# thomasantony/splat

Hardware: AMD Instinct MI355X
Metric: frames_per_sec (higher is better)
Workload: dtype f32

## Files before the change

### splat_amd/csrc/splat_api.hip

```cpp
#include <algorithm>
#include <cmath>
#include <cstdio>
#include <cstdlib>
#include <cstring>
#include <mutex>
#include <new>
#include <string>
#include <unordered_map>
#include <vector>

#include "splat_context.h"

using namespace splat;

static thread_local std::string g_create_error;
static std::mutex g_ledger_mu;
static std::unordered_map<void*, std::pair<splat_ctx*, size_t>> g_ledger;

namespace splat {
CommState** ctx_comm_slot(splat_ctx* c) { return &c->comm; }
hipStream_t ctx_stream(splat_ctx* c) { return c->stream; }
hipStream_t frame_stream(splat_ctx* c) { return (c->last_lane && c->comp2) ? c->comp2 : c->stream; }
int frame_tail(splat_ctx* c) {
    if (c->last_ring < 0 || !c->ring[c->last_ring].used) return SPLAT_OK;
// ... 502 lines not shown
            c->iters_alloc = m * 4u;
        }
        HIP_TRY(c, hipMemsetAsync(c->d_iters, 0, sizeof(uint2) * (size_t)m * 4u, cs));
        iters = c->d_iters;
        c->iters_valid = true;
    }
    CompositeArgs comp{};
    comp.s = cs; comp.knobs = &c->knobs; comp.n_tiles = m; comp.fc = c->fc; comp.recs = s.recs; comp.argb = d_argb; comp.status = f.d_st; comp.orig = c->orig;
    comp.fused_sort_max = retained ? 0u : c->fused_sort_max; comp.iters = iters; comp.keep_keys = want_iters || f.retain == SPLAT_RETAIN_WRITER;
    comp.pair_walk = pd.pair_walk != 0;
    comp.libm_exp = (c->cfg.mode & SPLAT_MODE_LIBM_EXP) != 0; comp.clear_first = c->clear_first;
    comp.lists = f.lists; comp.lists.near_m = pd.near_cap ? s.near_m : nullptr;
    comp.keys = f.keys; comp.keys.keys2 = pd.comp_sorts != 0 ? s.keys2 : nullptr;
    if (retained) {
        const bool near = c->ret_set.near_cap != 0u;
        comp.lists.near_m = near ? s.near_m : nullptr; comp.keys.keys2 = near ? s.keys2 : nullptr;
    }
    comp.hints = hint_table(c);
    if (c->knobs.dbg_stage_cache != 0u && f.retain == SPLAT_RETAIN_WRITER) {
        const size_t waves = (size_t)c->m_alloc * 4u;
        if (!c->stage_nv || !c->stage_mask) {
            dfree(c->stage_nv); dfree(c->stage_mask);
            HIP_TRY(c, dmalloc(c, &c->stage_nv, sizeof(unsigned int) * 2u * waves));
            HIP_TRY(c, dmalloc(c, &c->stage_mask, sizeof(unsigned long long) * 32u * waves));
        }
        HIP_TRY(c, hipMemsetAsync(c->stage_nv, 0, sizeof(unsigned int) * 2u * waves, cs));
        c->ret_set.frames = 0;
    }
    if (retained && c->knobs.dbg_stage_cache != 0u && c->stage_nv && c->stage_mask) {
        comp.stage_nv = c->stage_nv; comp.stage_mask = c->stage_mask;
        if (c->knobs.dbg_proven_starts != 0u && c->fc.close_width == 0.0f) comp.proven_start = c->proven_start();
        if (c->knobs.dbg_stage_cache == 2u && c->ret_set.frames >= 2u)
            HIP_TRY(c, hipMemsetAsync(c->stage_mask, 0, sizeof(unsigned long long) * 32u * (size_t)c->m_alloc * 4u, cs));
        c->ret_set.frames++;
    }
    comp.refine = c->fc.close_width == 0.0f ? pd.refine : 0u;
    launch_composite(comp);
    c->last_near = retained ? c->ret_set.near_cap != 0u : pd.near_cap != 0u;
    HIP_TRY(c, f.mark(6, cs));
    if (want_iters) HIP_TRY(c, hipMemcpyAsync(&c->h_status[f.r], f.d_st, sizeof(FrameStatus), hipMemcpyDeviceToHost, cs));
    HIP_TRY(c, hipEventRecord(f.ev->e[7], cs));
    return SPLAT_OK;
}

int decide_retention(splat_ctx* c, const splat_camera* cam, int* action) {
    splat_retain_input in;
    std::memset(&in, 0, sizeof in);
    static_assert(sizeof(splat_camera) + 2 * sizeof(int32_t) <= sizeof in.cam, "the camera and the slab fit the decision's words");
    std::memcpy(in.cam, cam, sizeof(splat_camera));
    const int32_t slab[2] = {c->slab0, c->slab1};
    std::memcpy(reinterpret_cast<unsigned char*>(in.cam) + sizeof(splat_camera), slab, sizeof slab);
    in.epoch = c->bin_epoch; in.still_frames = c->pol.still_frames;
    in.enabled = (c->retain_lists != 0 && c->knobs.dbg_ntiles == 0u) ? 1 : 0;
    in.overlap = c->overlap; in.one_pass = c->fc.bucket_cap ? 1 : 0;
    splat_retain_decision d;
    const int wr = c->ret_set.ring;
// ... 431 lines not shown
    option_from_env(c, SPLAT_OPT_HOST_ZERO_COPY, "SPLAT_HOST_ZERO_COPY", 0, 1);
    option_from_env(c, SPLAT_OPT_COUNT_FIRST, "SPLAT_COUNT_FIRST", 0, 2);
    if (const char* kg = std::getenv("SPLAT_KEYS_PER_GAUSSIAN")) {
        const int v = std::atoi(kg);
        c->keys_per_gaussian = v <= 0 ? 0u : (unsigned int)std::min(256, std::max(4, v));
        c->env_pinned |= 1u << SPLAT_OPT_KEYS_PER_GAUSSIAN;
    }
    option_from_env(c, SPLAT_OPT_LARGE_SPLAT_TILES, "SPLAT_LARGE_TILES", -1, 1048576);
    option_from_env(c, SPLAT_OPT_LARGE_LIST_MIN, "SPLAT_LARGE_LIST_MIN", -1, 1e9);
    option_from_env(c, SPLAT_OPT_START_REFINE, "SPLAT_START_REFINE", 0, 1);
    option_from_env(c, SPLAT_OPT_RETAIN_LISTS, "SPLAT_RETAIN", 0, 1);
    if (const char* lm = std::getenv("SPLAT_LAYOUT_MOTION")) c->layout_motion = std::atoi(lm) != 0 ? 1 : 0;
    if (const char* k1 = std::getenv("SPLAT_SORT_RADIX_MIN")) c->knobs.sort_radix_min = (unsigned int)std::max(0, std::atoi(k1));
    if (const char* k2 = std::getenv("SPLAT_SCAN_THREADS")) c->knobs.scan_threads = std::atoi(k2);
    if (const char* k3 = std::getenv("SPLAT_DBG_NTILES")) c->knobs.dbg_ntiles = (unsigned int)std::max(0, std::atoi(k3));
    if (const char* k8 = std::getenv("SPLAT_DBG_SELECT_STRIDE")) c->knobs.dbg_select_stride = (unsigned int)std::max(0, std::atoi(k8));
    if (const char* k10 = std::getenv("SPLAT_START_HINTS")) { c->start_hints = std::min(2, std::max(0, std::atoi(k10))); c->env_pinned |= 1u << SPLAT_OPT_START_HINTS; }
    if (const char* k7 = std::getenv("SPLAT_DBG_ONE_PASS_SELECT")) c->one_pass_select = std::atoi(k7) != 0;
    if (const char* k11 = std::getenv("SPLAT_DBG_KEYS2_ENTRIES")) c->knobs.dbg_keys2_entries = std::strtoull(k11, nullptr, 10);
    if (const char* k9 = std::getenv("SPLAT_DBG_HINT_RADIUS")) c->knobs.dbg_hint_radius = std::atoi(k9);
    if (const char* k12 = std::getenv("SPLAT_DBG_SELECT_BLIND")) c->knobs.dbg_select_blind = std::atoi(k12) != 0 ? 1u : 0u;
    if (const char* k15 = std::getenv("SPLAT_DBG_PROVEN_STARTS")) c->knobs.dbg_proven_starts = (unsigned int)std::min(2, std::max(0, std::atoi(k15)));
    if (const char* k14 = std::getenv("SPLAT_DBG_BRACKET_COUNT")) c->knobs.dbg_bracket_count = std::atoi(k14) != 0 ? 1u : 0u;
    if (const char* k13 = std::getenv("SPLAT_DBG_STAGE_CACHE")) c->knobs.dbg_stage_cache = (unsigned int)std::min(2, std::max(0, std::atoi(k13)));
    if (const char* k5 = std::getenv("SPLAT_DBG_STARTS")) c->knobs.dbg_starts = std::atoi(k5) != 0 ? 1u : 0u;
    if (const char* k4 = std::getenv("SPLAT_COMP_LDS_PAD")) c->knobs.comp_lds_pad = (unsigned int)std::max(0, std::atoi(k4));
    if (const char* k1p = std::getenv("SPLAT_K1_LDS_PAD")) c->knobs.k1_lds_pad = (unsigned int)std::min(48 * 1024, std::max(0, std::atoi(k1p)));
    auto bail = [&](const char* what, hipError_t err) {
        g_create_error = std::string(what) + ": " + hipGetErrorString(err);
        splat_destroy(c);
        return SPLAT_ERR_HIP;
    };
    if ((e = hipSetDevice(cfg->device)) != hipSuccess) return bail("hipSetDevice", e);
    if ((e = init_device_kernels()) != hipSuccess) return bail("hipFuncSetAttribute", e);
    if ((e = hipStreamCreateWithFlags(&c->stream, hipStreamNonBlocking)) != hipSuccess) return bail("hipStreamCreate", e);
    c->own_stream = true;
    {
        int lo = 0, hi = 0;
        (void)hipDeviceGetStreamPriorityRange(&lo, &hi);
        int prio = c->pipeline >= 6 ? (lo + hi) / 2 : hi;
        if (const char* ep = std::getenv("SPLAT_BIN_PRIO")) prio = std::atoi(ep) > 0 ? hi : (std::atoi(ep) < 0 ? lo : (lo + hi) / 2);
        if ((e = hipStreamCreateWithPriority(&c->bin_stream, hipStreamNonBlocking, prio)) != hipSuccess) return bail("hipStreamCreate", e);
        if ((e = hipStreamCreateWithPriority(&c->sort_stream, hipStreamNonBlocking, prio)) != hipSuccess) return bail("hipStreamCreate", e);
    }
    if (c->overlap >= 2 && c->pipeline) { if ((e = ensure_copy_stream(c)) != hipSuccess) return bail("hipStreamCreate", e); c->comp2 = c->copy_stream; }
    for (Slot& s : c->slots) {
// ... 624 lines not shown
```

### splat_amd/csrc/splat_context.h

```cpp
#ifndef SPLAT_CONTEXT_H
#define SPLAT_CONTEXT_H
#include <string>
#include <vector>

#include "splat_internal.h"
#include "../../include/splat_policy.h"
#include "../../include/splat_retain.h"

#define HIP_TRY(ctx, expr)                                                                             \
    do {                                                                                               \
        hipError_t _e = (expr);                                                                        \
        if (_e != hipSuccess) {                                                                        \
            (ctx)->err = std::string(#expr) + ": " + hipGetErrorString(_e);                            \
            return SPLAT_ERR_HIP;                                                                      \
        }                                                                                              \
    } while (0)

namespace splat {
constexpr int N_EV = 9;
constexpr int N_TIMES = 6;
constexpr int EV_RING = 32;
static_assert(EV_RING == SPLAT_POLICY_RING, "the frame policy sees the whole status ring");
constexpr int N_SLOTS = 4;

// ... 93 lines not shown
    uint64_t bucket_bytes = 128ull << 30;
    uint64_t layout_want = 0;
    unsigned int layout_m = 0;
    bool last_one_pass = false;
    unsigned int* zero_layout = nullptr;
    uint64_t dev_bytes = 0, dev_bytes_peak = 0;
    splat::LaunchKnobs knobs;
    float region_spare = 4.0f;
    uint64_t frame_idx = 0;
    uint64_t bin_idx = 0;
    int retain_lists = 1;
    uint64_t bin_epoch = 0;
    splat_retain_state ret{};
    uint64_t frames_retained = 0;
    struct RetainSet {
        int slot = -1, ring = -1;
        unsigned int near_cap = 0;
        splat::FrameStatus status{};
        unsigned int frames = 0;
    } ret_set;
    unsigned int* stage_nv = nullptr;
    unsigned long long* stage_mask = nullptr;
    unsigned int* proven_start() const { return stage_nv ? stage_nv + (size_t)m_alloc * 4u : nullptr; }
    int last_slot = -1;
    bool last_lists_in_memory = false;
    splat::FrameStatus* h_status = nullptr;
    splat::FrameStatus* d_status_ring = nullptr;
    bool clear_first = false;
    uint32_t* d_img = nullptr;
    size_t img_cap = 0;
    static constexpr int S_IMGS = 4;
    uint32_t* s_img[S_IMGS] = {};
    size_t s_cap = 0;
    hipStream_t copy_stream = nullptr;
    hipEvent_t s_rendered[S_IMGS] = {}, s_copied[S_IMGS] = {};
    const uint32_t* s_dst[S_IMGS] = {};
    bool s_used[S_IMGS] = {};
    uint64_t s_idx = 0;
    int s_ring[S_IMGS] = {-1, -1, -1, -1};
    splat_camera s_cam[S_IMGS] = {};
    int slab0 = 0, slab1 = -1;
    splat::EvSet ring[splat::EV_RING];
    int ring_next = 0;
    int last_ring = -1;
    double acc_ms[splat::N_TIMES] = {0, 0, 0, 0, 0, 0};
    uint64_t acc_frames = 0;
// ... 58 lines not shown
```

### splat_amd/csrc/splat_device_math.h

```cpp
#pragma once
#include <hip/hip_runtime.h>
#include <math.h>

__host__ __device__ __forceinline__ float reject_threshold(float opacity) {
    return (opacity > 0.0f) ? (logf(1.0f / (255.0f * opacity)) - 1e-3f)
                            : ((opacity <= 0.0f) ? 3.0e38f : -3.0e38f);
}

__host__ __device__ __forceinline__ bool any_sample_covered(float c, float h, float lo, float hi, float off) {
    float s1 = fminf(fmaxf(floorf(c - off) + off, lo), hi);
    float s2 = fminf(s1 + 1.0f, hi);
    return (int)(fabsf(s1 - c) <= h) | (int)(fabsf(s2 - c) <= h);
}

__device__ __forceinline__ float exp_neg(float x) {
    const float L2E_HI = __uint_as_float(0x3fb8aa3bu), L2E_LO = __uint_as_float(0x32a5705fu);
    const float LN2 = 0.6931471805599453f;
    float ph = x * L2E_HI;
    float pl = fmaf(x, L2E_HI, -ph);
    pl = fmaf(x, L2E_LO, pl);
    const float e = __builtin_amdgcn_exp2f(ph);
    return fmaf(e * pl, LN2, e);
}

// ... 44 lines not shown
    const unsigned long long ki = __builtin_bit_cast(unsigned long long, kd);
    kd -= SHIFT;
    const double r = fma(InvLn2N, xd, -kd);
    const double sc = __builtin_bit_cast(double, tab[ki & 31ull] + (ki << 47));
    const double zz = C0 * r + C1;
    const double r2 = r * r;
    double y = C2 * r + 1.0;
    y = zz * r2 + y;
    y = y * sc;
    return (float)y;
}
__host__ __device__ __forceinline__ float sigmoid_libm(float v) { return 1.0f / (1.0f + expf_libm_full(-v)); }

__host__ __device__ __forceinline__ float div255(float k) {
    const float RH = 0x1.010102p-8f, RL = -0x1.fdfdfep-33f;
    return fmaf(k, RH, k * RL);
}
__device__ __forceinline__ float blend_channel(float k, float ia, float ac) {
    const float x = __builtin_amdgcn_fmed3f(ia * div255(k) + ac, 0.0f, 1.0f);
    return truncf(x * 255.0f);
}

template <class E>
__device__ __forceinline__ float fragment_alpha(float sx, float sy, const float4& a, const float4& b, E e_of_power, bool& cov) {
    float dx = sx - a.x, dy = a.y - sy;
    cov = (fabsf(dx) <= a.z) & (fabsf(dy) <= a.w);
    float power = -0.5f * (b.x * dx * dx + b.z * dy * dy) - b.y * dx * dy;
    float alpha = fminf(0.99f, b.w * e_of_power(power));
    bool accept = cov & !(power > 0.0f) & !(alpha < 1.0f / 255.0f);
    return accept ? alpha : 0.0f;
}

typedef float f2 __attribute__((ext_vector_type(2)));
__device__ __forceinline__ f2 pk_add_clamp(f2 a, f2 b) {
    f2 r;
    asm("v_pk_add_f32 %0, %1, %2 clamp" : "=v"(r) : "v"(a), "v"(b));
    return r;
}
__device__ __forceinline__ f2 blend_channel2(f2 k, float ia, f2 ac) {
    const float RH = 0x1.010102p-8f, RL = -0x1.fdfdfep-33f;
    const f2 f = __builtin_elementwise_fma(k, (f2)(RH), k * RL);
    const f2 y = pk_add_clamp(ia * f, ac) * 255.0f;
    return (f2){truncf(y.x), truncf(y.y)};
}
__device__ __forceinline__ f2 exp_neg2(f2 power) {
    const float L2E_HI = __uint_as_float(0x3fb8aa3bu), L2E_LO = __uint_as_float(0x32a5705fu), LN2 = 0.6931471805599453f;
    const f2 ph = power * L2E_HI;
    f2 pl = __builtin_elementwise_fma(power, (f2)(L2E_HI), -ph);
    pl = __builtin_elementwise_fma(power, (f2)(L2E_LO), pl);
    const f2 e = {__builtin_amdgcn_exp2f(ph.x), __builtin_amdgcn_exp2f(ph.y)};
    return __builtin_elementwise_fma(e * pl, (f2)(LN2), e);
}
__device__ __forceinline__ f2 fragment_alpha2(f2 sx2, f2 sy2, f2 cx, f2 cy, const float4& h, f2 A, f2 C, f2 Bc, f2 op) {
// ... 11 lines not shown
```

### splat_amd/csrc/splat_internal.h

```cpp
#ifndef SPLAT_INTERNAL_H
#define SPLAT_INTERNAL_H
#include <hip/hip_runtime.h>
#include <stdint.h>

#include "../../include/splat_hip.h"

#ifndef SPLAT_K1X
#define SPLAT_K1X 0
#endif
#ifndef SPLAT_EXP_STAGE2
#define SPLAT_EXP_STAGE2 0
#endif
#ifndef SPLAT_EXP_NO_BRACKET
#define SPLAT_EXP_NO_BRACKET 0
#endif
#ifndef SPLAT_EXP_K1DUMMY
#define SPLAT_EXP_K1DUMMY 0
#endif
#ifndef SPLAT_EXP_SKIPFULL
#define SPLAT_EXP_SKIPFULL 0
#endif
#ifndef SPLAT_EXP_SORT2
#define SPLAT_EXP_SORT2 0
#endif
// ... 64 lines not shown
    unsigned long long layout_total;
};

struct Rec {
    float4 a;
    float4 b;
    float4 c;
};

struct LaunchKnobs {
    unsigned int sort_radix_min = 128;
    int scan_threads = 0;
    unsigned int dbg_ntiles = 0;
    unsigned int comp_lds_pad = 0;
    unsigned int k1_lds_pad = 0;
    unsigned int dbg_select_stride = 0;
    unsigned long long dbg_keys2_entries = 0;
    int dbg_hint_radius = -1;
    unsigned int dbg_select_blind = 0;
    unsigned int dbg_starts = 0;
    unsigned int dbg_bracket_count = 0;
    unsigned int dbg_proven_starts = 1;
    unsigned int dbg_stage_cache = 1;
};

struct HintTable {
    unsigned int* base;
    size_t stride;

    static constexpr unsigned int NEED_PLANE = 0u, NEED_PLANES = 4u;
    static constexpr unsigned int DEPTH_PLANE = NEED_PLANE + NEED_PLANES, DEPTH_PLANES = 1u;
    static constexpr unsigned int START_PLANE = DEPTH_PLANE + DEPTH_PLANES, START_PLANES = 4u;
    static constexpr unsigned int REFINE_PLANE = START_PLANE + START_PLANES, REFINE_PLANES = 4u;
    static constexpr unsigned int HINT_WORDS = 13u;
    static_assert(DEPTH_PLANE == 4u && START_PLANE == 5u && REFINE_PLANE == 9u && REFINE_PLANE + REFINE_PLANES == HINT_WORDS,
                  "the four parts tile the table exactly");

    unsigned int* plane(unsigned int k) const { return base ? base + k * stride : nullptr; }
    unsigned int* needs() const { return plane(NEED_PLANE); }
    unsigned int* select_depth() const { return plane(DEPTH_PLANE); }
    unsigned int* starts() const { return plane(START_PLANE); }
    unsigned int* refinement() const { return plane(REFINE_PLANE); }
    size_t words() const { return HINT_WORDS * stride; }
    size_t bytes() const { return sizeof(unsigned int) * words(); }
};

// ... 158 lines not shown
    unsigned int tiles_x, tile_rows;
    unsigned int grid;
    bool at_rest;
    int hint_radius;
};
void launch_select(const SelectArgs& a);

struct CompositeArgs {
    hipStream_t s; const LaunchKnobs* knobs; unsigned int n_tiles; FrameConst fc;
    TileLists lists;
    KeyBuffers keys;
    const Rec* recs; uint32_t* argb; FrameStatus* status; const unsigned int* orig;
    unsigned int fused_sort_max;
    uint2* iters;
    bool keep_keys;
    bool pair_walk;
    bool libm_exp;
    bool clear_first;
    HintTable hints;
    unsigned int refine;
    unsigned int* proven_start;
    unsigned int* stage_nv;
    unsigned long long* stage_mask;
};
void launch_composite(const CompositeArgs& a);
void launch_status_set(hipStream_t s, FrameStatus* status, const FrameStatus& v);
hipError_t init_device_kernels();

struct CommState;
CommState** ctx_comm_slot(splat_ctx* c);
hipStream_t ctx_stream(splat_ctx* c);
hipStream_t frame_stream(splat_ctx* c);
int ctx_device(const splat_ctx* c);
int frame_tail(splat_ctx* c);
int ctx_quiesce(splat_ctx* c);
int ctx_fail(splat_ctx* c, int code, const char* msg);
void comm_release(CommState* s);

}
#endif
```

### splat_amd/csrc/splat_kernels.hip

```cpp
#include <algorithm>
#include <cstddef>
#include <cstdlib>
#include <type_traits>

#include "splat_internal.h"
#include "splat_device_math.h"

namespace splat {
static constexpr unsigned long long KERNELS_EXP2F_TAB[32] = {
    0x3ff0000000000000ull, 0x3fefd9b0d3158574ull, 0x3fefb5586cf9890full, 0x3fef9301d0125b51ull, 0x3fef72b83c7d517bull,
    0x3fef54873168b9aaull, 0x3fef387a6e756238ull, 0x3fef1e9df51fdee1ull, 0x3fef06fe0a31b715ull, 0x3feef1a7373aa9cbull,
    0x3feedea64c123422ull, 0x3feece086061892dull, 0x3feebfdad5362a27ull, 0x3feeb42b569d4f82ull, 0x3feeab07dd485429ull,
    0x3feea47eb03a5585ull, 0x3feea09e667f3bcdull, 0x3fee9f75e8ec5f74ull, 0x3feea11473eb0187ull, 0x3feea589994cce13ull,
    0x3feeace5422aa0dbull, 0x3feeb737b0cdc5e5ull, 0x3feec49182a3f090ull, 0x3feed503b23e255dull, 0x3feee89f995ad3adull,
    0x3feeff76f2fb5e47ull, 0x3fef199bdd85529cull, 0x3fef3720dcef9069ull, 0x3fef5818dcfba487ull, 0x3fef7c97337b9b5full,
    0x3fefa4afa2a490daull, 0x3fefd0765b6e4540ull};
constexpr bool exp2f_tab_is_the_headers() {
    for (int i = 0; i < 32; ++i) if (KERNELS_EXP2F_TAB[i] != EXP2F_TAB_HOST[i]) return false;
    return true;
}
static_assert(exp2f_tab_is_the_headers(), "splat_kernels.hip's copy of EXP2F_TAB differs from splat_device_math.h's");
}


// ... 2239 lines not shown
            }
            __syncthreads();
        }
    };
    const unsigned int r1 = min(n, (unsigned int)CAP), r2 = min(n, 2u * CAP), r3 = min(n, 3u * CAP);
    unsigned long long* g = keys + base;
    unsigned long long* h = keys2 + off2[tile];
    merge(g, r1, g + r1, r2 - r1, h);
    merge(g + r2, r3 - r2, g + r3, n - r3, h + r2);
    __syncthreads();
    merge(h, r2, h + r2, n - r2, g);
}

__device__ __forceinline__ unsigned long long uniform_u64(unsigned long long v) {
    return ((unsigned long long)(unsigned int)__builtin_amdgcn_readfirstlane((int)(v >> 32)) << 32) |
           (unsigned long long)(unsigned int)__builtin_amdgcn_readfirstlane((int)(unsigned int)v);
}

struct WaveLds { float4 a[64]; float4 b[64]; float4 c[64]; };

#ifndef SPLAT_REFINE_MIN_STEP
#define SPLAT_REFINE_MIN_STEP 8
#endif
#ifndef SPLAT_COMP_WAVES
#define SPLAT_COMP_WAVES 1
#endif
struct CompArgs {
    FrameConst fc;
    const unsigned int* offsets; const unsigned int* order; const unsigned int* lens;
    unsigned long long* keys; const Rec* recs; uint32_t* argb; FrameStatus* status;
    unsigned int fused_sort_max, radix_min;
    uint2* iters;
    unsigned int keep_keys, clear_first;
    const unsigned int* orig;
    unsigned long long* keys2; const unsigned int* near_m;
    unsigned int* need_hint; unsigned int* start_hint; const unsigned int* off2;
    unsigned int* probe_hint;
    unsigned int refine;
    unsigned int* stage_nv; unsigned long long* stage_mask;
    unsigned int* proven_start;
};
typedef const __attribute__((address_space(4))) CompArgs* KernArgs;
template <bool PAIR, bool LIBM, bool KEEP>
static __device__ void repair_tile(KernArgs ka, unsigned int smem_lds, unsigned int exptab_lds, unsigned int item, bool again);

template <bool PAIR, bool LIBM, int LONGM, bool KEEP = false>
__device__ __forceinline__ void composite_tile(unsigned char* smem, const unsigned long long* exptab, const unsigned int item, const FrameConst& fc,
                                               const unsigned int* __restrict__ offsets, const unsigned int* __restrict__ order,
                                               const unsigned int* __restrict__ lens, unsigned long long* __restrict__ keys,
                                               const Rec* __restrict__ recs, uint32_t* __restrict__ argb,
                                               FrameStatus* __restrict__ status, unsigned int fused_sort_max,
                                               unsigned int radix_min, uint2* __restrict__ iters, unsigned int keep_keys,
                                               const unsigned int* __restrict__ orig, const unsigned int clear_first,
                                               unsigned long long* __restrict__ keys2, const unsigned int* __restrict__ near_m,
                                               unsigned int* __restrict__ need_hint, unsigned int* __restrict__ start_hint,
                                               const unsigned int* __restrict__ off2, KernArgs ka ,
                                               const bool walk_this_wave = true, const bool second_walk = false ) {
    auto late = [&]() -> KernArgs {
        unsigned long long p = (unsigned long long)(size_t)ka;
        asm volatile("" : "+s"(p));
        return (KernArgs)(size_t)p;
    };
    static_assert(sizeof(WaveLds) * 4 <= sort_lds_bytes<256, 2048>(), "staging fits the sort workspace");
    WaveLds* slds = reinterpret_cast<WaveLds*>(smem);
    const unsigned int tile = (unsigned int)__builtin_amdgcn_readfirstlane((int)order[item]);
    const unsigned int tid = threadIdx.x;
    const unsigned int beg = __builtin_amdgcn_readfirstlane(offsets[tile]);
    const unsigned int end = beg + __builtin_amdgcn_readfirstlane(lens[tile]);
    if (beg == end) {
        if (clear_first) {
            const KernArgs k = late();
            const int tiles_x = k->fc.tiles_x, W = k->fc.W, H = k->fc.H, r0 = k->fc.row_px0, r1 = k->fc.row_px1;
            const int txx0 = (int)(tile % (unsigned int)tiles_x), tyy0 = (int)(tile / (unsigned int)tiles_x) + k->fc.tile_row0;
            const int px0 = txx0 * TILE + (int)(tid & 15u), py0 = tyy0 * TILE + (int)(tid >> 4);
            if (px0 < W && py0 < H && py0 >= r0 && py0 < r1) k->argb[(size_t)py0 * W + px0] = 0u;
        }
        return;
    }
    unsigned int* const lds_idx = reinterpret_cast<unsigned int*>(smem + sizeof(WaveLds) * 4);
    static_assert(sizeof(WaveLds) * 4 + 2048 * 4 <= sort_lds_bytes<256, 2048>(), "the order fits behind the batches");
    static_assert(sizeof(WaveLds) * 4 + 2048 * 4 + 4 * 32 * 8 <= sort_lds_bytes<256, 2048>(), "the batch masks fit too");
    unsigned long long* const wmask = reinterpret_cast<unsigned long long*>(smem + sizeof(WaveLds) * 4 + 2048 * 4) + (tid >> 6) * 32u;
    bool own_order = end - beg >= 2u && end - beg <= fused_sort_max;
    unsigned int lb = beg;
    bool has_far = false;
    const unsigned long long* wk = keys;
    {
        const unsigned long long* gin = keys + beg;
        unsigned int n_sort = end - beg;
        if constexpr (LONGM == 1) {
            if (end - beg > 2048u) {
                (void)sort_long_list(smem, keys + beg, keys2 + off2[tile], end - beg, end - beg, radix_min, status, orig);
                __syncthreads();
            }
        }
        if constexpr (LONGM == 2) {
            if (end - beg > 2048u) {
                const unsigned int m = (unsigned int)__builtin_amdgcn_readfirstlane((int)near_m[tile]);
                if (m < end - beg) {
                    has_far = true; lb = end - m;
                    wk = keys2 + off2[tile] - lb;
                }
            }
        }
        if (own_order) {
// ... 31 lines not shown
    const float sxm = inside ? sx : __uint_as_float(0x7fc00000u), sym = inside ? sy : __uint_as_float(0x7fc00000u);

    auto fetch = [&](unsigned int base, unsigned int cnt, Rec& r) {
        if (lane < cnt) r = recs[own_order ? lds_idx[base - lb + lane] : (unsigned int)wk[base + lane]];
    };
    auto may_contribute = [&](const Rec& r) -> bool {
        const float a = r.b.x, b = r.b.y, c = r.b.z;
        const float ac = a * c;
        if (!(a > 0.0f && c > 0.0f && ac - b * b > 1e-3f * ac)) return true;
        const float x0 = xlo - r.a.x, x1 = xhi - r.a.x, y0 = r.a.y - yhi, y1 = r.a.y - ylo;
        auto q = [&](float x, float y) { return a * x * x + 2.0f * b * x * y + c * y * y; };
        auto cl = [](float v, float lo, float hi) { return fminf(fmaxf(v, lo), hi); };
        const float nbc = -b * __builtin_amdgcn_rcpf(c), nba = -b * __builtin_amdgcn_rcpf(a);
        const bool xin = x0 <= 0.0f && x1 >= 0.0f, yin = y0 <= 0.0f && y1 >= 0.0f;
        const float ex = (x0 > 0.0f) ? x0 : x1, ey = (y0 > 0.0f) ? y0 : y1;
        const float qv = q(ex, cl(nbc * ex, y0, y1)), qh = q(cl(nba * ey, x0, x1), ey);
        const float big = 3.0e38f;
        float qmin = fminf(xin ? big : qv, yin ? big : qh);
        if (xin && yin) qmin = 0.0f;
        const float pmax = -0.5f * qmin;
        return !(pmax + 1e-3f * (1.0f + fabsf(pmax)) < r.c.w);
    };
    auto stage = [&](const Rec& r, unsigned int cnt, unsigned int base, bool only_contributing, bool scan_layout = false,
                     bool pair_layout = false, int reuse_k = -1, unsigned int reuse_shift = 0u, int save_k = -1) -> unsigned int {
        __builtin_amdgcn_fence(__ATOMIC_RELEASE, "wavefront");
        __builtin_amdgcn_wave_barrier();
        bool ov = false;
        if (reuse_k >= 0) {
            ov = (((wmask[reuse_k] >> reuse_shift) >> lane) & 1ull) != 0ull;
        } else if (lane < cnt) {
            ov = any_sample_covered(r.a.x, r.a.z, xlo, xhi, off) && any_sample_covered(r.a.y, r.a.w, ylo, yhi, off);
            if (ov && only_contributing) ov = may_contribute(r);
#if SPLAT_EXP_STAGE2
            Rec r2 = r;
            asm volatile("" : "+v"(r2.a.x), "+v"(r2.a.y), "+v"(r2.b.x), "+v"(r2.b.y), "+v"(r2.c.w));
            bool ov2 = any_sample_covered(r2.a.x, r2.a.z, xlo, xhi, off) && any_sample_covered(r2.a.y, r2.a.w, ylo, yhi, off);
            if (ov2 && only_contributing) ov2 = may_contribute(r2);
            ov = ov & ov2;
#endif
        }
        const unsigned long long m = __builtin_amdgcn_ballot_w64(ov);
        if (save_k >= 0 && lane == 0u) wmask[save_k] = m;
        if (ov) {
            const unsigned int slot = __builtin_amdgcn_mbcnt_hi((unsigned int)(m >> 32), __builtin_amdgcn_mbcnt_lo((unsigned int)m, 0u));
            if (pair_layout) {
                float* P = reinterpret_cast<float*>(&L) + (slot >> 1) * 24u + (slot & 1u);
                P[0] = r.a.x; P[2] = r.a.y; P[4] = r.a.z; P[6] = r.a.w;
                P[8] = r.b.x; P[10] = r.b.z; P[12] = r.b.y; P[14] = r.b.w;
                float* Q = reinterpret_cast<float*>(&L) + (slot >> 1) * 24u + 2u * (slot & 1u);
                Q[16] = r.c.x; Q[17] = r.c.y; Q[20] = r.c.z;
            } else if (scan_layout) {
                const float L2E = 1.4426950408889634f;
                L.a[slot] = make_float4(r.a.x, r.a.y, __uint_as_float(base + lane), 0.0f);
                L.b[slot] = make_float4(-0.5f * L2E * r.b.x, -L2E * r.b.y, -0.5f * L2E * r.b.z, __log2f(r.b.w));
            } else {
                L.a[slot] = r.a; L.b[slot] = r.b;
                L.c[slot] = make_float4(r.c.x, r.c.y, r.c.z, __uint_as_float(base + lane));
            }
        }
        const unsigned int kk = (unsigned int)__builtin_popcountll(m);
        if (pair_layout && (kk & 1u) && lane == 0) {
            float* P = reinterpret_cast<float*>(&L) + (kk >> 1) * 24u + 1u;
            P[0] = 0.0f; P[2] = 0.0f; P[4] = -1.0f; P[6] = -1.0f; P[8] = 0.0f; P[10] = 0.0f; P[12] = 0.0f; P[14] = 0.0f;
            float* Q = reinterpret_cast<float*>(&L) + (kk >> 1) * 24u + 2u;
            Q[16] = 0.0f; Q[17] = 0.0f; Q[20] = 0.0f;
        }
        __builtin_amdgcn_fence(__ATOMIC_ACQUIRE, "wavefront");
        __builtin_amdgcn_wave_barrier();
        return kk;
    };
    auto expv = [&](float x) -> float {
        if constexpr (LIBM) return exp_libm(x, exptab);
        else return exp_neg(x);
    };

    bool need_far = false;
    unsigned int itA = 0, itB = 0;
    unsigned int nvc = 0xffffffffu;
    if constexpr (KEEP) {
        if (!second_walk) {
            const KernArgs kc = late();
            const unsigned int* const nv_l = kc->stage_nv;
            const unsigned long long kept = kc->stage_mask[(size_t)(tile * 4u + wave) * 32u + (lane & 31u)];
            nvc = min((unsigned int)__builtin_amdgcn_readfirstlane((int)nv_l[tile * 4u + wave]), 32u);
            __builtin_amdgcn_fence(__ATOMIC_RELEASE, "wavefront");
            __builtin_amdgcn_wave_barrier();
            if (lane < nvc) wmask[lane] = kept;
            __builtin_amdgcn_fence(__ATOMIC_ACQUIRE, "wavefront");
            __builtin_amdgcn_wave_barrier();
        }
    }
    float alast = -1.0f;
    if (!need_far) {
        bool found = !inside;
        Rec r;
        unsigned int cntN = min(64u, end - lb), bsN = end - cntN;
        fetch(bsN, cntN, r);
        while (true) {
            const unsigned int bs = bsN, cnt = cntN;
            const unsigned int k = stage(r, cnt, bs, false);
            if (bs > lb) { cntN = min(64u, bs - lb); bsN = bs - cntN; fetch(bsN, cntN, r); }
            unsigned int jsel = 0xffffffffu;
            for (unsigned int j = k; j-- > 0;) {
                const float4 a = L.a[j];
                const bool cov = (fabsf(sxm - a.x) <= a.z) & (fabsf(a.y - sym) <= a.w);
                jsel = (cov & !found) ? j : jsel;
                found = found | cov;
                if (__builtin_amdgcn_ballot_w64(!found) == 0ull) break;
            }
            if (__builtin_amdgcn_ballot_w64(jsel != 0xffffffffu) != 0ull) {
// ... 66 lines not shown
        if (ws == 0xffffffffu) ws = end;
    }
    const bool keeping = KEEP && nvc != 0xffffffffu && !scanned;
    if (keeping) nA = nvc;

    const float cw = fc.close_width;
    float R = (float)((old >> 16) & 0xffu), G = (float)((old >> 8) & 0xffu), B = (float)(old & 0xffu);
    float R2 = 255.0f, G2 = 255.0f, B2 = 255.0f;
    auto shade = [&](auto BRt, const float4& a, const float4& b, const float4& c) {
        constexpr bool BR = decltype(BRt)::value;
        bool cov;
        const float alpha = fragment_alpha(sxm, sym, a, b, expv, cov);
        const float ia = 1.0f - alpha;
        const float ar = alpha * c.x, ag = alpha * c.y, ab = alpha * c.z;
        R = blend_channel(R, ia, ar);
        G = blend_channel(G, ia, ag);
        B = blend_channel(B, ia, ab);
        if (BR) {
            R2 = blend_channel(R2, ia, ar);
            G2 = blend_channel(G2, ia, ag);
            B2 = blend_channel(B2, ia, ab);
        }
    };
    const f2 sxm2 = {sxm, sxm}, sym2 = {sym, sym};
    auto shade_pair = [&](auto BRt, const float4& q0, const float4& q1, const float4& q2, const float4& q3, const float4& q4,
                          const float4& q5) {
        constexpr bool BR = decltype(BRt)::value;
        const f2 cx = {q0.x, q0.y}, cy = {q0.z, q0.w}, A = {q2.x, q2.y}, C = {q2.z, q2.w}, Bc = {q3.x, q3.y}, op = {q3.z, q3.w};
        const f2 alpha = fragment_alpha2(sxm2, sym2, cx, cy, q1, A, C, Bc, op);
        const float alpha0 = alpha.x, alpha1 = alpha.y;
        auto blend_one = [&](float alpha, f2 rg, float b) {
            const float ia = 1.0f - alpha;
            const f2 arg = alpha * rg;
            const float ab = alpha * b;
            f2 s = blend_channel2((f2){R, G}, ia, arg);
            R = s.x; G = s.y;
            B = blend_channel(B, ia, ab);
            if (BR) {
                s = blend_channel2((f2){R2, G2}, ia, arg);
                R2 = s.x; G2 = s.y;
                B2 = blend_channel(B2, ia, ab);
            }
        };
        blend_one(alpha0, (f2){q4.x, q4.y}, q5.x);
        blend_one(alpha1, (f2){q4.z, q4.w}, q5.z);
    };
    auto run = [&](auto BRt, unsigned int start) -> unsigned int {
        constexpr bool BR = decltype(BRt)::value;
        Rec r;
        unsigned int kb = start < end ? (end - 1u - start) >> 6 : 0u;
        unsigned int bsN = start, cntN = start < end ? (end - (kb << 6)) - start : 0u;
        if (cntN) fetch(bsN, cntN, r);
        while (cntN) {
            const unsigned int bs = bsN, cnt = cntN;
            const bool reuse = kb < nA;
            const unsigned int abase = (end - lb >= ((kb + 1u) << 6)) ? end - ((kb + 1u) << 6) : lb;
            const bool keep = KEEP && keeping && !reuse && kb < 32u && bs == abase;
            const unsigned int k = stage(r, cnt, bs, true, false, PAIR, reuse ? (int)kb : -1, bs - abase, keep ? (int)kb : -1);
            bsN = bs + cnt; cntN = min(64u, end - bsN); kb -= cntN ? 1u : 0u;
            if (cntN) fetch(bsN, cntN, r);
            if constexpr (PAIR) {
                const float4* P4 = reinterpret_cast<const float4*>(&L);
                for (unsigned int j = 0; j < (k + 1u) / 2u; ++j)
                    shade_pair(BRt, P4[6 * j], P4[6 * j + 1], P4[6 * j + 2], P4[6 * j + 3], P4[6 * j + 4], P4[6 * j + 5]);
            } else {
                for (unsigned int j = 0; j < k; ++j) shade(BRt, L.a[j], L.b[j], L.c[j]);
            }
            itB += k;
            if (BR && __builtin_amdgcn_ballot_w64(inside & ((R2 - R > cw) | (G2 - G > cw) | (B2 - B > cw))) == 0ull) return bsN;
        }
        return end;
    };
    unsigned int start = ws;
    if constexpr (KEEP) {
        if (cw == 0.0f && hinted && probe == 0u && !second_walk && start > lb) {
            const KernArgs kp = late();
            const unsigned int* const pv_l = kp->proven_start;
            if (pv_l != nullptr && (unsigned int)__builtin_amdgcn_readfirstlane((int)pv_l[tile * 4u + wave]) == end - start) probe = 0x20000000u;
        }
    }
    while (!need_far) {
        if (start <= lb) {
            if (has_far) { need_far = true; break; }
            R = (float)((old >> 16) & 0xffu); G = (float)((old >> 8) & 0xffu); B = (float)(old & 0xffu);
            run(std::false_type{}, lb);
            break;
        }
// ... 14 lines not shown
        if (!open) {
            R = truncf((R + R2) * 0.5f); G = truncf((G + G2) * 0.5f); B = truncf((B + B2) * 0.5f);
            if (pos < end) run(std::false_type{}, pos);
            if constexpr (KEEP) probe = (probe & 0x20000000u) ? 0u : (probe | 0x40000000u);
            break;
        }
        if (probe != 0u && !(probe >> 31)) {
            probe |= 0x80000000u;
            const KernArgs kr = late();
            const unsigned int g = (unsigned int)__builtin_amdgcn_readfirstlane((int)kr->start_hint[tile * 4u + wave]);
            if (lane == 0) atomicAdd(&kr->status->n_probe_fail, 1u);
            if (g > end - start && g < end - lb) { start = end - g; continue; }
        }
        if (lane == 0) atomicAdd(&late()->status->n_fallback, 1ull);
        const unsigned int depth = end - start;
        start = (start - lb > depth) ? start - depth : lb;
    }
    const float A = (alast < 0.0f) ? (float)(old >> 24) : truncf(alast * 255.0f);
    const KernArgs kl = late();
    uint2* const iters_l = kl->iters;
    if (iters_l != nullptr && lane == 0) {
        const unsigned int kk = kl->keep_keys;
        uint2 v = (kk & 2u) ? make_uint2(end - beg, end - max(start, beg)) : make_uint2(itA, itB);
        if (second_walk && !(kk & 2u)) { const uint2 o = iters_l[item * 4u + wave]; v.x += o.x; v.y += o.y; }
        iters_l[item * 4u + wave] = v;
    }
    if constexpr (LONGM != 0) {
        unsigned int* const need_l = kl->need_hint;
        if (need_l != nullptr && end - beg > 2048u && lane == 0u) need_l[tile * 4u + wave] = need_far ? 0xffffffffu : end - max(start, lb);
    }
    unsigned int* const start_l = kl->start_hint;
    if (start_l != nullptr && early && !need_far && (scanned || start != ws) && lane == 0u) {
        unsigned int used = max(end - max(start, lb), 1u);
        if (!has_far && used > (end - beg) - ((end - beg) >> 2)) used = end - beg;
        start_l[tile * 4u + wave] = used;
    }
    const unsigned int closed_here = KEEP ? probe & 0x40000000u : 0u;
    if constexpr (KEEP) probe &= 0x8000ffffu;
    if (probe != 0u && lane == 0u) {
        const bool failed = (probe >> 31) != 0u;
        const unsigned int half = (probe & 0xffffu) >> 1;
        const unsigned int step = failed ? (half >= (unsigned int)SPLAT_REFINE_MIN_STEP ? half : 0u) : probe;
        if (!failed) start_l[tile * 4u + wave] = end - ws;
        kl->probe_hint[tile * 4u + wave] = (kl->refine & 0xffff0000u) | step;
    }
    if constexpr (KEEP) {
        unsigned int* const pv_l = kl->proven_start;
        if (closed_here != 0u && !need_far && pv_l != nullptr && lane == 0u) pv_l[tile * 4u + wave] = end - start;
    }
    if (KEEP && keeping && !need_far && max(start, lb) < end) {
        const unsigned int s = max(start, lb), kf = (end - 1u - s) >> 6;
        const unsigned int ab = (end - lb >= ((kf + 1u) << 6)) ? end - ((kf + 1u) << 6) : lb;
        const unsigned int nv_new = min(kf + (s == ab ? 1u : 0u), 32u);
        unsigned int* const nv_l = kl->stage_nv;
        const unsigned int nv_old = (unsigned int)__builtin_amdgcn_readfirstlane((int)nv_l[tile * 4u + wave]);
        if (nv_new > nv_old) {
            __builtin_amdgcn_fence(__ATOMIC_RELEASE, "wavefront");
            __builtin_amdgcn_wave_barrier();
            if (lane >= nv_old && lane < nv_new) kl->stage_mask[(size_t)(tile * 4u + wave) * 32u + lane] = wmask[lane];
            if (lane == 0u) nv_l[tile * 4u + wave] = nv_new;
            __builtin_amdgcn_fence(__ATOMIC_ACQUIRE, "wavefront");
            __builtin_amdgcn_wave_barrier();
        }
    }
    if (need_far) return true;
    if (inside)
        kl->argb[(size_t)py * kl->fc.W + px] = ((uint32_t)A << 24) | ((uint32_t)R << 16) | ((uint32_t)G << 8) | (uint32_t)B;
    return false;
    };
    if constexpr (LONGM != 2) {
        (void)walk_list();
    } else {
        const bool again = walk_list();
        if (has_far && __syncthreads_or(again ? 1 : 0) != 0) {
            if (tid == 0u) atomicAdd(&late()->status->n_near_fallback, 1u);
            repair_tile<PAIR, LIBM, KEEP>(ka, (unsigned int)(size_t)(__attribute__((address_space(3))) unsigned char*)smem,
                                    (unsigned int)(size_t)(__attribute__((address_space(3))) const unsigned long long*)exptab, item, again);
        }
    }
}

template <bool PAIR, bool LIBM, bool KEEP>
// ... 297 lines not shown
    if (!n_tiles) return;
    const unsigned int* off2 = a.lists.off2;
    if (!off2) off2 = a.lists.offsets;
    int hint_radius = a.hint_radius;
    unsigned int grid = a.grid;
    if (a.knobs->dbg_hint_radius >= 0) hint_radius = a.knobs->dbg_hint_radius;
    if (a.knobs->dbg_select_stride) grid = (n_tiles + a.knobs->dbg_select_stride - 1u) / a.knobs->dbg_select_stride;
    if (!grid) grid = (n_tiles + 7u) / 8u;
    hipLaunchKernelGGL(select_near_kernel, dim3(std::min(grid, n_tiles)), dim3(256), 0, a.s, a.lists.offsets, a.lists.order, a.lists.lens, a.keys.keys, a.keys.keys2, a.status, a.orig, a.knobs->sort_radix_min,
                       std::min(std::max(a.near_cap, 64u), 2048u), a.need_hint, a.lists.near_m, a.tiles_x, a.tile_rows, a.near_thr, n_tiles, a.at_rest ? 1u : 0u, off2, std::min(std::max(hint_radius, 0), 7), a.knobs->dbg_select_blind);
}
void launch_composite(const CompositeArgs& c) {
    unsigned int n_tiles = c.n_tiles;
    if (!n_tiles) return;
    const unsigned int* off2 = c.lists.off2;
    if (!off2) off2 = c.lists.offsets;
    if (c.knobs->dbg_ntiles) n_tiles = std::min(n_tiles, c.knobs->dbg_ntiles);
    const unsigned int pad = c.knobs->comp_lds_pad;
    unsigned long long* keys2 = c.keys.keys2;
    const unsigned int* near_m = c.lists.near_m;
    unsigned int *need_hint = c.hints.needs(), *start_hint = c.hints.starts(), *probe_hint = c.hints.refinement();
    const bool near = near_m != nullptr && keys2 != nullptr && need_hint != nullptr;
    const unsigned int flags = (c.keep_keys ? 1u : 0u) | (c.knobs->dbg_starts ? 2u : 0u) | (c.knobs->dbg_bracket_count ? 4u : 0u) |
                               (c.knobs->dbg_proven_starts == 2u ? 8u : 0u);
    CompArgs a;
    a.fc = c.fc; a.offsets = c.lists.offsets; a.order = c.lists.order; a.lens = c.lists.lens; a.keys = c.keys.keys; a.recs = c.recs; a.argb = c.argb; a.status = c.status;
    a.fused_sort_max = c.fused_sort_max; a.radix_min = c.knobs->sort_radix_min; a.iters = c.iters; a.keep_keys = flags; a.clear_first = c.clear_first ? 1u : 0u;
    a.orig = c.orig; a.keys2 = keys2; a.near_m = near_m; a.need_hint = near ? need_hint : nullptr; a.start_hint = start_hint; a.off2 = off2;
    a.probe_hint = probe_hint; a.refine = (probe_hint != nullptr && start_hint != nullptr) ? c.refine : 0u;
    const bool keep_verdicts = c.stage_nv != nullptr && c.stage_mask != nullptr && (near || keys2 == nullptr);
    a.stage_nv = keep_verdicts ? c.stage_nv : nullptr; a.stage_mask = keep_verdicts ? c.stage_mask : nullptr;
    a.proven_start = (keep_verdicts && c.fc.close_width == 0.0f) ? c.proven_start : nullptr;
    auto go = [&](auto kern) { hipLaunchKernelGGL(kern, dim3(n_tiles), dim3(256), pad, c.s, a); };
    if (keep_verdicts && near) {
        if (c.libm_exp) go(composite_retained_kernel<false, true, 2>);
        else if (c.pair_walk) go(composite_retained_kernel<true, false, 2>);
        else go(composite_retained_kernel<false, false, 2>);
    } else if (keep_verdicts) {
        if (c.libm_exp) go(composite_retained_kernel<false, true, 0>);
        else if (c.pair_walk) go(composite_retained_kernel<true, false, 0>);
        else go(composite_retained_kernel<false, false, 0>);
    } else if (near) {
        if (c.libm_exp) go(composite_exact_kernel<false, true, 2>);
        else if (c.pair_walk) go(composite_exact_kernel<true, false, 2>);
        else go(composite_exact_kernel<false, false, 2>);
    } else if (keys2 != nullptr) {
        if (c.libm_exp) go(composite_exact_kernel<false, true, 1>);
        else if (c.pair_walk) go(composite_exact_kernel<true, false, 1>);
        else go(composite_exact_kernel<false, false, 1>);
    } else {
        if (c.libm_exp) go(composite_exact_kernel<false, true, 0>);
        else if (c.pair_walk) go(composite_exact_kernel<true, false, 0>);
        else go(composite_exact_kernel<false, false, 0>);
    }
}
// ... 3 lines not shown
```

Measured before the change: 5651.

## Cache per-batch fully-accepted splat masks to skip coverage tests in retained compositing

On the retained-list composite path, each batch now records which staged splats were accepted by every pixel in the wave, using ballot masks, and stores those masks in a second half of the stage_mask buffer. On later frames, splats marked fully accepted are blended with a simplified alpha computation that skips the coverage, power and alpha threshold checks. This is meant to cut per-fragment ALU and branch work in the compositing inner loop. It costs an extra per-wave LDS mask, extra global reads and writes, and a doubled stage_mask allocation, and it relies on the cached verdicts staying valid while the camera moves.

```diff
diff --git a/splat_amd/csrc/splat_api.hip b/splat_amd/csrc/splat_api.hip
--- a/splat_amd/csrc/splat_api.hip
+++ b/splat_amd/csrc/splat_api.hip
@@ -548,7 +548,7 @@
         if (!c->stage_nv || !c->stage_mask) {
             dfree(c->stage_nv); dfree(c->stage_mask);
             HIP_TRY(c, dmalloc(c, &c->stage_nv, sizeof(unsigned int) * 2u * waves));
-            HIP_TRY(c, dmalloc(c, &c->stage_mask, sizeof(unsigned long long) * 32u * waves));
+            HIP_TRY(c, dmalloc(c, &c->stage_mask, sizeof(unsigned long long) * 2u * 32u * waves));
         }
         HIP_TRY(c, hipMemsetAsync(c->stage_nv, 0, sizeof(unsigned int) * 2u * waves, cs));
         c->ret_set.frames = 0;
@@ -558,6 +558,9 @@
         if (c->knobs.dbg_proven_starts != 0u && c->fc.close_width == 0.0f) comp.proven_start = c->proven_start();
         if (c->knobs.dbg_stage_cache == 2u && c->ret_set.frames >= 2u)
             HIP_TRY(c, hipMemsetAsync(c->stage_mask, 0, sizeof(unsigned long long) * 32u * (size_t)c->m_alloc * 4u, cs));
+        if (c->knobs.dbg_full_steps != 0u) comp.stage_full = c->stage_full();
+        if (c->knobs.dbg_full_steps == 2u && c->ret_set.frames >= 2u)
+            HIP_TRY(c, hipMemsetAsync(c->stage_full(), 0xff, sizeof(unsigned long long) * 32u * (size_t)c->m_alloc * 4u, cs));
         c->ret_set.frames++;
     }
     comp.refine = c->fc.close_width == 0.0f ? pd.refine : 0u;
@@ -1035,6 +1038,8 @@
     if (const char* k12 = std::getenv("SPLAT_DBG_SELECT_BLIND")) c->knobs.dbg_select_blind = std::atoi(k12) != 0 ? 1u : 0u;
     if (const char* k15 = std::getenv("SPLAT_DBG_PROVEN_STARTS")) c->knobs.dbg_proven_starts = (unsigned int)std::min(2, std::max(0, std::atoi(k15)));
     if (const char* k14 = std::getenv("SPLAT_DBG_BRACKET_COUNT")) c->knobs.dbg_bracket_count = std::atoi(k14) != 0 ? 1u : 0u;
+    if (const char* k17 = std::getenv("SPLAT_DBG_FULL_COUNT")) c->knobs.dbg_full_count = std::atoi(k17) != 0 ? 1u : 0u;
+    if (const char* k16 = std::getenv("SPLAT_DBG_FULL_STEPS")) c->knobs.dbg_full_steps = (unsigned int)std::min(2, std::max(0, std::atoi(k16)));
     if (const char* k13 = std::getenv("SPLAT_DBG_STAGE_CACHE")) c->knobs.dbg_stage_cache = (unsigned int)std::min(2, std::max(0, std::atoi(k13)));
     if (const char* k5 = std::getenv("SPLAT_DBG_STARTS")) c->knobs.dbg_starts = std::atoi(k5) != 0 ? 1u : 0u;
     if (const char* k4 = std::getenv("SPLAT_COMP_LDS_PAD")) c->knobs.comp_lds_pad = (unsigned int)std::max(0, std::atoi(k4));
diff --git a/splat_amd/csrc/splat_context.h b/splat_amd/csrc/splat_context.h
--- a/splat_amd/csrc/splat_context.h
+++ b/splat_amd/csrc/splat_context.h
@@ -139,6 +139,7 @@
     unsigned int* stage_nv = nullptr;
     unsigned long long* stage_mask = nullptr;
     unsigned int* proven_start() const { return stage_nv ? stage_nv + (size_t)m_alloc * 4u : nullptr; }
+    unsigned long long* stage_full() const { return stage_mask ? stage_mask + (size_t)m_alloc * 4u * 32u : nullptr; }
     int last_slot = -1;
     bool last_lists_in_memory = false;
     splat::FrameStatus* h_status = nullptr;
diff --git a/splat_amd/csrc/splat_device_math.h b/splat_amd/csrc/splat_device_math.h
--- a/splat_amd/csrc/splat_device_math.h
+++ b/splat_amd/csrc/splat_device_math.h
@@ -90,13 +90,35 @@
 }
 
 template <class E>
-__device__ __forceinline__ float fragment_alpha(float sx, float sy, const float4& a, const float4& b, E e_of_power, bool& cov) {
+__host__ __device__ __forceinline__ float fragment_alpha(float sx, float sy, const float4& a, const float4& b, E e_of_power, bool& cov, bool& accept) {
     float dx = sx - a.x, dy = a.y - sy;
     cov = (fabsf(dx) <= a.z) & (fabsf(dy) <= a.w);
     float power = -0.5f * (b.x * dx * dx + b.z * dy * dy) - b.y * dx * dy;
     float alpha = fminf(0.99f, b.w * e_of_power(power));
-    bool accept = cov & !(power > 0.0f) & !(alpha < 1.0f / 255.0f);
+    accept = cov & !(power > 0.0f) & !(alpha < 1.0f / 255.0f);
     return accept ? alpha : 0.0f;
+}
+template <class E>
+__host__ __device__ __forceinline__ float fragment_alpha(float sx, float sy, const float4& a, const float4& b, E e_of_power, bool& cov) {
+    bool accept;
+    return fragment_alpha(sx, sy, a, b, e_of_power, cov, accept);
+}
+template <class E>
+__device__ __forceinline__ float fragment_alpha_mask(float sx, float sy, const float4& a, const float4& b, E e_of_power, unsigned long long& accept_mask) {
+    float dx = sx - a.x, dy = a.y - sy;
+    const bool cx = fabsf(dx) <= a.z, cy = fabsf(dy) <= a.w;
+    float power = -0.5f * (b.x * dx * dx + b.z * dy * dy) - b.y * dx * dy;
+    float alpha = fminf(0.99f, b.w * e_of_power(power));
+    const bool np = !(power > 0.0f), na = !(alpha < 1.0f / 255.0f);
+    accept_mask = __builtin_amdgcn_ballot_w64(cx) & __builtin_amdgcn_ballot_w64(cy) & __builtin_amdgcn_ballot_w64(np) & __builtin_amdgcn_ballot_w64(na);
+    bool accept = cx & cy & np & na;
+    return accept ? alpha : 0.0f;
+}
+template <class E>
+__host__ __device__ __forceinline__ float fragment_alpha_accepted(float sx, float sy, const float4& a, const float4& b, E e_of_power) {
+    float dx = sx - a.x, dy = a.y - sy;
+    float power = -0.5f * (b.x * dx * dx + b.z * dy * dy) - b.y * dx * dy;
+    return fminf(0.99f, b.w * e_of_power(power));
 }
 
 typedef float f2 __attribute__((ext_vector_type(2)));
diff --git a/splat_amd/csrc/splat_internal.h b/splat_amd/csrc/splat_internal.h
--- a/splat_amd/csrc/splat_internal.h
+++ b/splat_amd/csrc/splat_internal.h
@@ -110,6 +110,8 @@
     unsigned int dbg_bracket_count = 0;
     unsigned int dbg_proven_starts = 1;
     unsigned int dbg_stage_cache = 1;
+    unsigned int dbg_full_steps = 1;
+    unsigned int dbg_full_count = 0;
 };
 
 struct HintTable {
@@ -314,6 +316,7 @@
     unsigned int* proven_start;
     unsigned int* stage_nv;
     unsigned long long* stage_mask;
+    unsigned long long* stage_full;
 };
 void launch_composite(const CompositeArgs& a);
 void launch_status_set(hipStream_t s, FrameStatus* status, const FrameStatus& v);
diff --git a/splat_amd/csrc/splat_kernels.hip b/splat_amd/csrc/splat_kernels.hip
--- a/splat_amd/csrc/splat_kernels.hip
+++ b/splat_amd/csrc/splat_kernels.hip
@@ -2285,6 +2285,9 @@
 #ifndef SPLAT_REFINE_MIN_STEP
 #define SPLAT_REFINE_MIN_STEP 8
 #endif
+#ifndef SPLAT_FULL_WALK
+#define SPLAT_FULL_WALK 1
+#endif
 #ifndef SPLAT_COMP_WAVES
 #define SPLAT_COMP_WAVES 1
 #endif
@@ -2302,6 +2305,7 @@
     unsigned int refine;
     unsigned int* stage_nv; unsigned long long* stage_mask;
     unsigned int* proven_start;
+    unsigned long long* stage_full;
 };
 typedef const __attribute__((address_space(4))) CompArgs* KernArgs;
 template <bool PAIR, bool LIBM, bool KEEP>
@@ -2344,6 +2348,7 @@
     static_assert(sizeof(WaveLds) * 4 + 2048 * 4 <= sort_lds_bytes<256, 2048>(), "the order fits behind the batches");
     static_assert(sizeof(WaveLds) * 4 + 2048 * 4 + 4 * 32 * 8 <= sort_lds_bytes<256, 2048>(), "the batch masks fit too");
     unsigned long long* const wmask = reinterpret_cast<unsigned long long*>(smem + sizeof(WaveLds) * 4 + 2048 * 4) + (tid >> 6) * 32u;
+    unsigned long long* const wfull = reinterpret_cast<unsigned long long*>(lds_idx) + (tid >> 6) * 32u;
     bool own_order = end - beg >= 2u && end - beg <= fused_sort_max;
     unsigned int lb = beg;
     bool has_far = false;
@@ -2421,7 +2426,8 @@
         return !(pmax + 1e-3f * (1.0f + fabsf(pmax)) < r.c.w);
     };
     auto stage = [&](const Rec& r, unsigned int cnt, unsigned int base, bool only_contributing, bool scan_layout = false,
-                     bool pair_layout = false, int reuse_k = -1, unsigned int reuse_shift = 0u, int save_k = -1) -> unsigned int {
+                     bool pair_layout = false, int reuse_k = -1, unsigned int reuse_shift = 0u, int save_k = -1,
+                     unsigned long long fullw = 0ull ) -> unsigned int {
         __builtin_amdgcn_fence(__ATOMIC_RELEASE, "wavefront");
         __builtin_amdgcn_wave_barrier();
         bool ov = false;
@@ -2454,7 +2460,8 @@
                 L.b[slot] = make_float4(-0.5f * L2E * r.b.x, -L2E * r.b.y, -0.5f * L2E * r.b.z, __log2f(r.b.w));
             } else {
                 L.a[slot] = r.a; L.b[slot] = r.b;
-                L.c[slot] = make_float4(r.c.x, r.c.y, r.c.z, __uint_as_float(base + lane));
+                if constexpr (KEEP && !PAIR) L.c[slot] = make_float4(r.c.x, r.c.y, r.c.z, __uint_as_float((unsigned int)(fullw >> lane) & 1u));
+                else L.c[slot] = make_float4(r.c.x, r.c.y, r.c.z, __uint_as_float(base + lane));
             }
         }
         const unsigned int kk = (unsigned int)__builtin_popcountll(m);
@@ -2475,16 +2482,19 @@
 
     bool need_far = false;
     unsigned int itA = 0, itB = 0;
+    unsigned int itF = 0;
     unsigned int nvc = 0xffffffffu;
     if constexpr (KEEP) {
         if (!second_walk) {
             const KernArgs kc = late();
             const unsigned int* const nv_l = kc->stage_nv;
             const unsigned long long kept = kc->stage_mask[(size_t)(tile * 4u + wave) * 32u + (lane & 31u)];
+            const unsigned long long* const full_l = PAIR ? nullptr : kc->stage_full;
+            const unsigned long long keptf = full_l != nullptr ? full_l[(size_t)(tile * 4u + wave) * 32u + (lane & 31u)] : 0ull;
             nvc = min((unsigned int)__builtin_amdgcn_readfirstlane((int)nv_l[tile * 4u + wave]), 32u);
             __builtin_amdgcn_fence(__ATOMIC_RELEASE, "wavefront");
             __builtin_amdgcn_wave_barrier();
-            if (lane < nvc) wmask[lane] = kept;
+            if (lane < nvc) { wmask[lane] = kept; if constexpr (!PAIR) wfull[lane] = keptf; }
             __builtin_amdgcn_fence(__ATOMIC_ACQUIRE, "wavefront");
             __builtin_amdgcn_wave_barrier();
         }
@@ -2597,6 +2607,19 @@
             B2 = blend_channel(B2, ia, ab);
         }
     };
+    auto blend_in = [&](auto BRt, const float alpha, const float4& c) {
+        constexpr bool BR = decltype(BRt)::value;
+        const float ia = 1.0f - alpha;
+        const float ar = alpha * c.x, ag = alpha * c.y, ab = alpha * c.z;
+        R = blend_channel(R, ia, ar);
+        G = blend_channel(G, ia, ag);
+        B = blend_channel(B, ia, ab);
+        if (BR) {
+            R2 = blend_channel(R2, ia, ar);
+            G2 = blend_channel(G2, ia, ag);
+            B2 = blend_channel(B2, ia, ab);
+        }
+    };
     const f2 sxm2 = {sxm, sxm}, sym2 = {sym, sym};
     auto shade_pair = [&](auto BRt, const float4& q0, const float4& q1, const float4& q2, const float4& q3, const float4& q4,
                           const float4& q5) {
@@ -2631,13 +2654,70 @@
             const bool reuse = kb < nA;
             const unsigned int abase = (end - lb >= ((kb + 1u) << 6)) ? end - ((kb + 1u) << 6) : lb;
             const bool keep = KEEP && keeping && !reuse && kb < 32u && bs == abase;
-            const unsigned int k = stage(r, cnt, bs, true, false, PAIR, reuse ? (int)kb : -1, bs - abase, keep ? (int)kb : -1);
+            const unsigned int kbc = kb;
+            unsigned long long fullw = 0ull;
+            if constexpr (KEEP && !PAIR) { if (reuse && keeping) fullw = wfull[kbc] >> (bs - abase); }
+            const unsigned int k = stage(r, cnt, bs, true, false, PAIR, reuse ? (int)kb : -1, bs - abase, keep ? (int)kb : -1, fullw);
             bsN = bs + cnt; cntN = min(64u, end - bsN); kb -= cntN ? 1u : 0u;
             if (cntN) fetch(bsN, cntN, r);
             if constexpr (PAIR) {
                 const float4* P4 = reinterpret_cast<const float4*>(&L);
                 for (unsigned int j = 0; j < (k + 1u) / 2u; ++j)
                     shade_pair(BRt, P4[6 * j], P4[6 * j + 1], P4[6 * j + 2], P4[6 * j + 3], P4[6 * j + 4], P4[6 * j + 5]);
+            } else if constexpr (KEEP) {
+#if SPLAT_EXP_FULL_ALL
+                if constexpr (!BR) { for (unsigned int j = 0; j < k; ++j) blend_in(BRt, fragment_alpha_accepted(sxm, sym, L.a[j], L.b[j], expv), L.c[j]); }
+                else
+#endif
+                {
+                unsigned long long fm = 0ull;
+                if (reuse && keeping) {
+                    fm = __builtin_amdgcn_ballot_w64(lane < k && __float_as_uint(L.c[lane].w) != 0u);
+                    itF += (unsigned int)__builtin_popcountll(fm);
+                }
+#if SPLAT_FULL_WALK == 1
+                if (keep) {
+                    for (unsigned int j = 0; j < k; ++j) {
+                        unsigned long long acc;
+                        blend_in(BRt, fragment_alpha_mask(sxm, sym, L.a[j], L.b[j], expv, acc), L.c[j]);
+                        if (acc == ~0ull) fm |= 1ull << j;
+                    }
+                } else {
+                    for (unsigned int j = 0; j < k;) {
+                        const unsigned long long t = fm >> j;
+                        const unsigned int e = t != 0ull ? j + (unsigned int)__builtin_ctzll(t) : k;
+                        for (; j < e; ++j) shade(BRt, L.a[j], L.b[j], L.c[j]);
+                        if (j == k) break;
+                        const unsigned long long u = ~(fm >> j);
+                        const unsigned int e2 = u != 0ull ? min(k, j + (unsigned int)__builtin_ctzll(u)) : k;
+                        for (; j < e2; ++j) blend_in(BRt, fragment_alpha_accepted(sxm, sym, L.a[j], L.b[j], expv), L.c[j]);
+                    }
+                }
+#else
+                for (unsigned int j = 0; j < k; ++j) {
+                    typedef float nf4 __attribute__((ext_vector_type(4)));
+                    typedef const __attribute__((address_space(3))) nf4* LdsRec;
+                    unsigned int pj = (unsigned int)(size_t)(LdsRec)reinterpret_cast<const nf4*>(&L.a[j]);
+                    asm("" : "+v"(pj));
+                    const LdsRec P = (LdsRec)(size_t)pj;
+                    const nf4 a4 = P[0], b4 = P[64], c4 = P[128];
+                    const float4 a = make_float4(a4.x, a4.y, a4.z, a4.w), b = make_float4(b4.x, b4.y, b4.z, b4.w), c = make_float4(c4.x, c4.y, c4.z, c4.w);
+                    if ((fm >> j) & 1ull) {
+                        blend_in(BRt, fragment_alpha_accepted(sxm, sym, a, b, expv), c);
+                    } else {
+                        unsigned long long acc;
+                        blend_in(BRt, fragment_alpha_mask(sxm, sym, a, b, expv, acc), c);
+                        if (acc == ~0ull) fm |= 1ull << j;
+                    }
+                }
+#endif
+                if (keep) {
+                    const unsigned long long m = wmask[kbc];
+                    const unsigned int slot = __builtin_amdgcn_mbcnt_hi((unsigned int)(m >> 32), __builtin_amdgcn_mbcnt_lo((unsigned int)m, 0u));
+                    const unsigned long long w = __builtin_amdgcn_ballot_w64((((m >> lane) & 1ull) != 0ull) && (((fm >> slot) & 1ull) != 0ull));
+                    if (lane == 0u) wfull[kbc] = w;
+                }
+                }
             } else {
                 for (unsigned int j = 0; j < k; ++j) shade(BRt, L.a[j], L.b[j], L.c[j]);
             }
@@ -2698,6 +2778,7 @@
     if (iters_l != nullptr && lane == 0) {
         const unsigned int kk = kl->keep_keys;
         uint2 v = (kk & 2u) ? make_uint2(end - beg, end - max(start, beg)) : make_uint2(itA, itB);
+        if (KEEP && (kk & 16u)) v.x = itF;
         if (second_walk && !(kk & 2u)) { const uint2 o = iters_l[item * 4u + wave]; v.x += o.x; v.y += o.y; }
         iters_l[item * 4u + wave] = v;
     }
@@ -2733,7 +2814,10 @@
         if (nv_new > nv_old) {
             __builtin_amdgcn_fence(__ATOMIC_RELEASE, "wavefront");
             __builtin_amdgcn_wave_barrier();
-            if (lane >= nv_old && lane < nv_new) kl->stage_mask[(size_t)(tile * 4u + wave) * 32u + lane] = wmask[lane];
+            if (lane >= nv_old && lane < nv_new) {
+                kl->stage_mask[(size_t)(tile * 4u + wave) * 32u + lane] = wmask[lane];
+                if constexpr (!PAIR) { unsigned long long* const full_l = kl->stage_full; if (full_l != nullptr) full_l[(size_t)(tile * 4u + wave) * 32u + lane] = wfull[lane]; }
+            }
             if (lane == 0u) nv_l[tile * 4u + wave] = nv_new;
             __builtin_amdgcn_fence(__ATOMIC_ACQUIRE, "wavefront");
             __builtin_amdgcn_wave_barrier();
@@ -3077,7 +3161,7 @@
     unsigned int *need_hint = c.hints.needs(), *start_hint = c.hints.starts(), *probe_hint = c.hints.refinement();
     const bool near = near_m != nullptr && keys2 != nullptr && need_hint != nullptr;
     const unsigned int flags = (c.keep_keys ? 1u : 0u) | (c.knobs->dbg_starts ? 2u : 0u) | (c.knobs->dbg_bracket_count ? 4u : 0u) |
-                               (c.knobs->dbg_proven_starts == 2u ? 8u : 0u);
+                               (c.knobs->dbg_proven_starts == 2u ? 8u : 0u) | (c.knobs->dbg_full_count ? 16u : 0u);
     CompArgs a;
     a.fc = c.fc; a.offsets = c.lists.offsets; a.order = c.lists.order; a.lens = c.lists.lens; a.keys = c.keys.keys; a.recs = c.recs; a.argb = c.argb; a.status = c.status;
     a.fused_sort_max = c.fused_sort_max; a.radix_min = c.knobs->sort_radix_min; a.iters = c.iters; a.keep_keys = flags; a.clear_first = c.clear_first ? 1u : 0u;
@@ -3086,6 +3170,7 @@
     const bool keep_verdicts = c.stage_nv != nullptr && c.stage_mask != nullptr && (near || keys2 == nullptr);
     a.stage_nv = keep_verdicts ? c.stage_nv : nullptr; a.stage_mask = keep_verdicts ? c.stage_mask : nullptr;
     a.proven_start = (keep_verdicts && c.fc.close_width == 0.0f) ? c.proven_start : nullptr;
+    a.stage_full = keep_verdicts ? c.stage_full : nullptr;
     auto go = [&](auto kern) { hipLaunchKernelGGL(kern, dim3(n_tiles), dim3(256), pad, c.s, a); };
     if (keep_verdicts && near) {
         if (c.libm_exp) go(composite_retained_kernel<false, true, 2>);
```

Measured after the change: 5593. -1.0%, worse.
